# HarborYuan/PolyphonicFormer

Hardware: AMD Instinct MI355X
Metric: frames/sec kernel-update+mask fwd, 1024x2048 N=153 S=3 (higher is better)
Workload: dtype bf16 (feature planes as given; query side: updator half hi/lo bf16, attention / FFN / towers one fp16 plane; one fp16 plane of dynamic kernels, fp16 logits); 1 GPU; cfg2: KernelUpdateIterHead.simple_test_mask_preds, 1024x2048, stride-8 128x256, N=153, S=3, L=133, random-init weights; hip_graph=True, streams=4, feature_input_dtype=bf16, mask_logit_input_dtype=float16, output_dtype=torch.float16, parallelism=frames sharded over 1 GPU(s), no data-path collective

## Files before the change

### polyphonicformer_amd/csrc/ph_convup.hip

```cpp
#include <stdlib.h>

#include <type_traits>

#include "ph_conv_inl.h"

__device__ __forceinline__ void lds_wait_all() {
    asm volatile("s_waitcnt lgkmcnt(0)" ::: "memory");
    __builtin_amdgcn_sched_barrier(0);
}


template <typename OutT> struct UpElem;
template <> struct UpElem<ph_h16> { static constexpr int E = PH_E_F16; };
template <> struct UpElem<uint16_t> { static constexpr int E = PH_E_BF16; };

template <int NRT> struct UpmCfg {
    static constexpr int NW = NRT + 1;
    static constexpr int TILEB = 256 * CONV_T * 2;
    static constexpr int ROWT = 128 + 16;
    static constexpr int TB = 32 * ROWT;
    static constexpr int PATCHB = NRT * 2 * TB;
    static constexpr int KBB = NRT * 32 * 4;
    static constexpr int CONSTB = 6 * 1024;
    static constexpr int NBUF = 3 * TILEB + PATCHB + KBB + CONSTB <= 160 * 1024 ? 3 : 2;
    static constexpr int LDSB = NBUF * TILEB + PATCHB + KBB + CONSTB;
};

template <int OFF> __device__ __forceinline__ void lds_write64_asm(uint32_t byte_addr, uint32_t lo, uint32_t hi) {
    const u32x2_t v = {lo, hi};
    asm volatile("ds_write_b64 %0, %1 offset:%2" ::"v"(byte_addr), "v"(v), "n"(OFF) : "memory");
}

template <int EO> __device__ __forceinline__ uint4 upm_main_frag(int lane, float w) {
    const int opx = lane & 31, g = lane >> 5, j = opx >> 1;
    uint32_t h[8];
#pragma unroll
    for (int e = 0; e < 8; ++e) {
        const int px = (e & 3) + 8 * (e >> 2) + 4 * g;
        float u = 0.f;
        if (px == j) u = 0.75f;
        else if ((opx & 1) ? px == j + 1 : px == j - 1) u = 0.25f;
        h[e] = f2e<EO>(w * u);
    }
    return make_uint4(pack2(h[0], h[1]), pack2(h[2], h[3]), pack2(h[4], h[5]), pack2(h[6], h[7]));
}
template <int EO> __device__ __forceinline__ uint4 upm_edge_frag(int lane, float wP, float wC) {
    const int opx = lane & 31, g = lane >> 5;
    const float l = (g == 0 && opx == 0) ? 0.25f : 0.f, r = (g == 0 && opx == 31) ? 0.25f : 0.f;
    return make_uint4(pack2(f2e<EO>(wP * l), f2e<EO>(wP * r)), pack2(f2e<EO>(wC * l), f2e<EO>(wC * r)), 0u, 0u);
}

template <int E, int NRT, int NTR, bool LOWRES, typename OutT>
__global__ __launch_bounds__(((NRT + 1) * 64)) void k_dynconv_up2m(const uint16_t* __restrict__ planes, const uint16_t* __restrict__ kern,
                                                                  int64_t kern_batch_stride, const float* __restrict__ kbias,
                                                                  int64_t kbias_batch_stride, OutT* __restrict__ logits_out,
                                                                  OutT* __restrict__ up_out, int B, int N, int H) {
    using C = UpmCfg<NRT>;
    constexpr int NBUF = C::NBUF, W = NTR * 64, ROWT = C::ROWT, EO = UpElem<OutT>::E, NH = 2 * NTR;
    constexpr bool COOP = E == PH_E_F16_FROM_BF16;
    extern __shared__ __attribute__((aligned(16))) uint16_t lds[];
    const int tid = threadIdx.x, lane = tid & 63;
    const int wave = __builtin_amdgcn_readfirstlane(tid >> 6);
    const bool producer = wave == NRT;
    const int rt = producer ? 0 : wave;
    const int g = lane >> 5, i16 = lane & 15, gi = (lane >> 4) & 1, ql = lane & 31;
    const int64_t HW = (int64_t)H * W;
    const int ntiles = H * NTR;

    const int64_t rows_total = (int64_t)B * H;
    const int R0 = (int)(rows_total * blockIdx.x / gridDim.x), R1 = (int)(rows_total * (blockIdx.x + 1) / gridDim.x);
    if (R0 >= R1) return;
    const int halo = (R0 % H) != 0 ? 1 : 0;
    const int tg0 = (R0 - halo) * NTR, tg1 = R1 * NTR;

    const uint32_t dma_lane_off = 2u * (uint32_t)((lane >> 3) * HW + (((lane & 7) ^ conv_swz(lane >> 3)) * 8));
    const int64_t row8_bytes = 2 * 8 * HW;
    const int64_t frame_jump = 2 * ((int64_t)PH_C * HW - (int64_t)ntiles * CONV_T);
    int it = tg0 % ntiles, ti = tg0;
    const char* iptr = (const char*)planes + 2 * ((int64_t)(tg0 / ntiles) * PH_C * HW + (int64_t)it * CONV_T);
    auto issue_next = [&](int buf) {
        const char* src = iptr + dma_lane_off;
#pragma unroll
        for (int j = 0; j < 32; ++j)
            __builtin_amdgcn_global_load_lds((const __attribute__((address_space(1))) void*)(src + j * row8_bytes),
                                             (PH_LDS void*)((PH_LDS char*)lds + buf * C::TILEB + j * 1024), 16, 0, PH_CPOL_STREAM);
        ++ti;
        iptr += 2 * CONV_T;
        if (++it == ntiles) { it = 0; iptr += frame_jump; }
    };
    if (producer) {
#pragma unroll
        for (int d = 0; d < NBUF - 1; ++d)
            if (ti < tg1) issue_next(d);
    }

    const int row0 = g * 8 + (i16 >> 2);
    uint32_t frag_off[2];
#pragma unroll
    for (int h = 0; h < 2; ++h) frag_off[h] = 2u * (uint32_t)(row0 * CONV_T + (((h * 4 + gi * 2) ^ conv_swz(row0)) * 8) + (i16 & 3) * 4);
    const uint32_t lds0 = lds_addr(lds);
    const uint32_t tbuf = lds0 + NBUF * C::TILEB + rt * 2 * C::TB;
    float* kb_lds = (float*)((unsigned char*)lds + NBUF * C::TILEB + C::PATCHB) + rt * 32;
    const uint32_t kb_addr = lds_addr(kb_lds) + 4 * ql;
    const uint32_t tw_addr = tbuf + (uint32_t)(ql * ROWT + 8 * g);
    const int sq = lane >> 3, ss = lane & 7;
    const uint32_t tr_addr = tbuf + (uint32_t)(sq * ROWT + 16 * ss);
    const int64_t up_plane = (int64_t)2 * H * 2 * W;
    const uint32_t up_lane_off = 2u * (uint32_t)(sq * up_plane + 8 * ss);
    const int64_t up_kk_bytes = 2 * 8 * up_plane;
    const uint32_t lr_lane_off = 2u * (uint32_t)(sq * HW + 8 * ss);
    const int64_t lr_kk_bytes = 2 * 8 * HW;

    const uint32_t cfrag = lds0 + NBUF * C::TILEB + C::PATCHB + C::KBB + 16u * (uint32_t)lane;
    if (wave == 0) {
        uint4* cw = (uint4*)((unsigned char*)lds + NBUF * C::TILEB + C::PATCHB + C::KBB) + lane;
        cw[0 * 64] = upm_main_frag<EO>(lane, 0.75f);
        cw[1 * 64] = upm_main_frag<EO>(lane, 0.25f);
        cw[2 * 64] = upm_edge_frag<EO>(lane, 0.75f, 0.25f);
        cw[3 * 64] = upm_edge_frag<EO>(lane, 0.25f, 0.75f);
        cw[4 * 64] = upm_main_frag<EO>(lane, 1.0f);
        cw[5 * 64] = upm_edge_frag<EO>(lane, 0.f, 1.0f);
    }
    __syncthreads();

    uint4 af[1][16];
    uint4 prev[NTR][2][2];
#pragma unroll
    for (int a = 0; a < NTR; ++a)
#pragma unroll
        for (int h = 0; h < 2; ++h) { prev[a][h][0] = make_uint4(0, 0, 0, 0); prev[a][h][1] = make_uint4(0, 0, 0, 0); }
    uint4 Cp0 = make_uint4(0, 0, 0, 0), Cp1 = Cp0;
    uint32_t Pe = 0, Ce = 0;

    auto mf = [&](uint4 a, uint4 b, f32x16_t c) -> f32x16_t {
        if constexpr (EO == PH_E_F16) return __builtin_amdgcn_mfma_f32_32x32x16_f16(__builtin_bit_cast(f16x8_t, a), __builtin_bit_cast(f16x8_t, b), c, 0, 0, 0);
        else return mfma32(a, b, c);
    };
    auto xg = [&](uint32_t v) -> uint32_t { return (uint32_t)__shfl_xor((int)v, 32); };
    const f32x16_t zero16 = {0.f, 0.f, 0.f, 0.f, 0.f, 0.f, 0.f, 0.f, 0.f, 0.f, 0.f, 0.f, 0.f, 0.f, 0.f, 0.f};

    auto out_row = [&](auto mp_tag, auto mc_tag, auto me_tag, uint4 P0, uint4 P1, uint4 C0, uint4 C1, uint4 e0, uint4 e1, char* dst_row) {
        constexpr int MP = decltype(mp_tag)::value, MC = decltype(mc_tag)::value, ME = decltype(me_tag)::value;
        uint32_t cf = cfrag;
        asm volatile("" : "+v"(cf));
        u32x4_t kc = lds_read128o_asm<MC * 1024>(cf), ke = lds_read128o_asm<ME * 1024>(cf), kp = kc;
        if constexpr (MP >= 0) kp = lds_read128o_asm<MP * 1024>(cf);
        lds_wait_all();
        const uint4 KC = __builtin_bit_cast(uint4, kc), KE = __builtin_bit_cast(uint4, ke), KP = __builtin_bit_cast(uint4, kp);
        f32x16_t a0 = zero16, a1 = zero16;
        if constexpr (MP >= 0) { a0 = mf(KP, P0, a0); a1 = mf(KP, P1, a1); }
        a0 = mf(KC, C0, a0); a1 = mf(KC, C1, a1);
        a0 = mf(KE, e0, a0); a1 = mf(KE, e1, a1);
        {
            uint32_t w[8];
#pragma unroll
            for (int j = 0; j < 8; ++j) w[j] = f2e_pk<EO>(a0[2 * j], a0[2 * j + 1]);
            lds_write64_asm<0>(tw_addr, w[0], w[1]);  lds_write64_asm<16>(tw_addr, w[2], w[3]);
            lds_write64_asm<32>(tw_addr, w[4], w[5]); lds_write64_asm<48>(tw_addr, w[6], w[7]);
#pragma unroll
            for (int j = 0; j < 8; ++j) w[j] = f2e_pk<EO>(a1[2 * j], a1[2 * j + 1]);
            lds_write64_asm<64>(tw_addr, w[0], w[1]); lds_write64_asm<80>(tw_addr, w[2], w[3]);
            lds_write64_asm<96>(tw_addr, w[4], w[5]); lds_write64_asm<112>(tw_addr, w[6], w[7]);
        }
        lds_wait_all();
        uint32_t tr = tr_addr;
        asm volatile("" : "+v"(tr));
        u32x4_t x[4];
        x[0] = lds_read128o_asm<0 * 8 * ROWT>(tr); x[1] = lds_read128o_asm<1 * 8 * ROWT>(tr);
        x[2] = lds_read128o_asm<2 * 8 * ROWT>(tr); x[3] = lds_read128o_asm<3 * 8 * ROWT>(tr);
        lds_wait_all();
#pragma unroll
        for (int kk = 0; kk < 4; ++kk)
            if (rt * 32 + sq + 8 * kk < N) st_nt16(dst_row + kk * up_kk_bytes + up_lane_off, __builtin_bit_cast(uint4, x[kk]));
    };
    int cur = 0, cur_b = -1;
    for (int gr = R0 - halo; gr < R1; ++gr) {
        const int b = gr / H, r = gr - b * H;
        const bool silent = gr < R0, first = r == 0, last = r == H - 1;
        if (!producer && b != cur_b) {
            const uint16_t* kr = kern + (int64_t)b * kern_batch_stride + (rt * 32 + (lane & 31)) * PH_C + g * 8;
#pragma unroll
            for (int ks = 0; ks < 16; ++ks) af[0][ks] = *(const uint4*)(kr + ks * 16);
            if (lane < 32) kb_lds[lane] = kbias[(int64_t)b * kbias_batch_stride + rt * 32 + lane];
            __builtin_amdgcn_s_waitcnt(0x0F70);
        }
        cur_b = b;
        char* up_row = (char*)(up_out + ((int64_t)b * N + rt * 32) * up_plane + (int64_t)(2 * r) * (2 * W));
        char* lr_row = LOWRES ? (char*)(logits_out + ((int64_t)b * N + rt * 32) * HW + (int64_t)r * W) : nullptr;

        auto emit = [&](auto eh_tag, uint4 P0, uint4 P1, uint4 C0, uint4 C1, uint32_t lP, uint32_t lC, uint32_t rP, uint32_t rC) {
            constexpr int EH = decltype(eh_tag)::value;
            uint32_t l0P, l0C, r1P, r1C;
            if constexpr (EH == 0) { l0P = P0.x & 0xFFFFu; l0C = C0.x & 0xFFFFu; }
            else { l0P = xg(lP) >> 16; l0C = xg(lC) >> 16; }
            if constexpr (EH == NH - 1) { r1P = xg(P1.w) >> 16; r1C = xg(C1.w) >> 16; }
            else { r1P = rP & 0xFFFFu; r1C = rC & 0xFFFFu; }
            const uint32_t p15 = xg(P0.w) >> 16, c15 = xg(C0.w) >> 16;
            const uint32_t keep = g ? 0u : 0xFFFFFFFFu;
            const uint4 e0 = make_uint4((l0P | (P1.x << 16)) & keep, (l0C | (C1.x << 16)) & keep, 0u, 0u);
            const uint4 e1 = make_uint4((p15 | (r1P << 16)) & keep, (c15 | (r1C << 16)) & keep, 0u, 0u);
            char* ub = up_row + 2 * 64 * EH;
            constexpr auto c0 = std::integral_constant<int, 0>{}; constexpr auto c1 = std::integral_constant<int, 1>{};
            constexpr auto c2 = std::integral_constant<int, 2>{}; constexpr auto c3 = std::integral_constant<int, 3>{};
            constexpr auto c4 = std::integral_constant<int, 4>{}; constexpr auto c5 = std::integral_constant<int, 5>{};
            constexpr auto cn = std::integral_constant<int, -1>{};
            if (!first) {
                out_row(c0, c1, c2, P0, P1, C0, C1, e0, e1, ub - 2 * (2 * W));
                out_row(c1, c0, c3, P0, P1, C0, C1, e0, e1, ub);
            } else {
                out_row(cn, c4, c5, P0, P1, C0, C1, e0, e1, ub);
            }
            if (last) out_row(cn, c4, c5, P0, P1, C0, C1, e0, e1, ub + 2 * (2 * W));
        };

        auto tile = [&](auto tc_tag) {
            constexpr int TC = decltype(tc_tag)::value;
            const int tg = gr * NTR + TC;
            if (producer) {
                const int younger = (tg1 - 1 - tg) < (NBUF - 2) ? (tg1 - 1 - tg) : (NBUF - 2);
                if (NBUF >= 3 && younger >= 1) asm volatile("s_waitcnt vmcnt(32)" ::: "memory");
                else asm volatile("s_waitcnt vmcnt(0)" ::: "memory");
            }
            __builtin_amdgcn_s_barrier();
            __builtin_amdgcn_sched_barrier(0);
            if (producer && ti < tg1) {
                int nb = cur + NBUF - 1;
                if (nb >= NBUF) nb -= NBUF;
                issue_next(nb);
            }
            __builtin_amdgcn_sched_barrier(0);
            if constexpr (COOP) {
                constexpr int PIECES = 256 * CONV_T * 2 / 16, LANES = C::NW * 64, ROUNDS = (PIECES + LANES - 1) / LANES;
                const uint32_t tb = lds0 + cur * C::TILEB + 16u * (uint32_t)tid;
                u32x4_t cv[ROUNDS];
#pragma unroll
                for (int q = 0; q < ROUNDS; ++q)
                    if ((q + 1) * LANES <= PIECES || tid < PIECES - q * LANES) cv[q] = lds_read128_asm(tb + q * LANES * 16);
                asm volatile("s_waitcnt lgkmcnt(0)" ::: "memory");
                __builtin_amdgcn_sched_barrier(0);
#pragma unroll
                for (int q = 0; q < ROUNDS; ++q)
                    if ((q + 1) * LANES <= PIECES || tid < PIECES - q * LANES) {
                        const uint4 h16 = bf2h_x8(__builtin_bit_cast(uint4, cv[q]));
                        lds_write128_asm(tb + q * LANES * 16, __builtin_bit_cast(u32x4_t, h16));
                    }
                asm volatile("s_waitcnt lgkmcnt(0)" ::: "memory");
                __builtin_amdgcn_s_barrier();
                __builtin_amdgcn_sched_barrier(0);
            }
            if (!producer) {
                float bl;
                asm volatile("ds_read_b32 %0, %1\n s_waitcnt lgkmcnt(0)" : "=&v"(bl) : "v"(kb_addr) : "memory");
                float bias[16];
#pragma unroll
                for (int q = 0; q < 16; ++q) bias[q] = bl;
#pragma unroll
                for (int h = 0; h < 2; ++h) {
                    const uint32_t fa = lds0 + cur * C::TILEB + frag_off[h];
                    f32x16_t acc;
                    constexpr int KB = 2;
                    u32x2_t bq[2][1][KB][2];
                    conv_read_batch<1, KB, 0>(fa, bq[0]);
                    conv_batches<1, 1, E, KB, 0, true>(fa, af, bq, acc, bias);
                    const uint4 cu0 = make_uint4(f2e_pk<EO>(acc[0], acc[1]), f2e_pk<EO>(acc[2], acc[3]), f2e_pk<EO>(acc[4], acc[5]), f2e_pk<EO>(acc[6], acc[7]));
                    const uint4 cu1 = make_uint4(f2e_pk<EO>(acc[8], acc[9]), f2e_pk<EO>(acc[10], acc[11]), f2e_pk<EO>(acc[12], acc[13]), f2e_pk<EO>(acc[14], acc[15]));
                    if (!silent) {
                        auto body = [&](auto hh_tag) {
                            constexpr int HH = decltype(hh_tag)::value;
                            if constexpr (LOWRES) {
                                asm volatile("s_nop 7" ::: "memory");
                                constexpr int HB = (HH & 1) * 64;
                                lds_write64_asm<C::TB + HB + 0>(tw_addr, cu0.x, cu0.y);  lds_write64_asm<C::TB + HB + 16>(tw_addr, cu0.z, cu0.w);
                                lds_write64_asm<C::TB + HB + 32>(tw_addr, cu1.x, cu1.y); lds_write64_asm<C::TB + HB + 48>(tw_addr, cu1.z, cu1.w);
                                if constexpr ((HH & 1) == 1) {
                                    lds_wait_all();
                                    u32x4_t x[4];
                                    x[0] = lds_read128o_asm<C::TB + 0 * 8 * ROWT>(tr_addr); x[1] = lds_read128o_asm<C::TB + 1 * 8 * ROWT>(tr_addr);
                                    x[2] = lds_read128o_asm<C::TB + 2 * 8 * ROWT>(tr_addr); x[3] = lds_read128o_asm<C::TB + 3 * 8 * ROWT>(tr_addr);
                                    lds_wait_all();
#pragma unroll
                                    for (int kk = 0; kk < 4; ++kk)
                                        if (rt * 32 + sq + 8 * kk < N)
                                            *(uint4*)(lr_row + 2 * 64 * TC + kk * lr_kk_bytes + lr_lane_off) = __builtin_bit_cast(uint4, x[kk]);
                                }
                            }
                            constexpr int TCp = (HH > 0) ? (HH - 1) / 2 : 0, hp = (HH > 0) ? (HH - 1) % 2 : 0;
                            if constexpr (HH > 0) {
                                emit(std::integral_constant<int, HH - 1>{}, prev[TCp][hp][0], prev[TCp][hp][1], Cp0, Cp1, Pe, Ce, prev[TC][h][0].x, cu0.x);
                                Pe = prev[TCp][hp][1].w; Ce = Cp1.w;
                                prev[TCp][hp][0] = Cp0; prev[TCp][hp][1] = Cp1;
                            }
                            if constexpr (HH == NH - 1) {
                                emit(std::integral_constant<int, HH>{}, prev[TC][h][0], prev[TC][h][1], cu0, cu1, Pe, Ce, 0u, 0u);
                                prev[TC][h][0] = cu0; prev[TC][h][1] = cu1;
                            } else {
                                Cp0 = cu0; Cp1 = cu1;
                            }
                        };
                        if (h == 0) body(std::integral_constant<int, 2 * TC>{});
                        else body(std::integral_constant<int, 2 * TC + 1>{});
                    } else {
                        prev[TC][h][0] = cu0; prev[TC][h][1] = cu1;
                    }
                }
            }
            cur = cur + 1 == NBUF ? 0 : cur + 1;
        };
        tile(std::integral_constant<int, 0>{});
        if constexpr (NTR > 1) tile(std::integral_constant<int, 1>{});
        if constexpr (NTR > 2) tile(std::integral_constant<int, 2>{});
        if constexpr (NTR > 3) tile(std::integral_constant<int, 3>{});
    }
}

extern "C" int ph_dynconv_up2_supported(int N, int H, int W, int prec, int out_dtype) {
    if (N <= 64 || N > 224 || H <= 0 || W != 256) return 0;
    if (((int64_t)H * W) % 128) return 0;
    if (prec == PH_PREC_BF16) return out_dtype == PH_OUT_BF16;
    if (prec == PH_PREC_F16 || prec == PH_PREC_BF16_KF16) return out_dtype == PH_OUT_F16;
    return 0;
}

template <int E, int NRT, typename OutT>
static void launch_up(const uint16_t* planes, const uint16_t* kern, int64_t kbs, const float* kbias, int64_t bbs, void* logits_out,
                      void* up_out, int B, int N, int H, int want_wgs, const PhUp2Knobs& kn, hipStream_t s) {
    constexpr int NTR = 4;
    const int64_t rows = (int64_t)B * H;
    int wgs = want_wgs > 0 ? want_wgs : ph_num_cus();
    if (wgs <= 0) wgs = 256;
    if (kn.wgs > 0) wgs = kn.wgs;
    if (wgs > rows) wgs = (int)rows;
    const dim3 grid(wgs), block((NRT + 1) * 64);
    constexpr int lds = UpmCfg<NRT>::LDSB;
#define UP_GO(LR)                                                                                                             \
    do {                                                                                                                      \
        static const bool once = [] {                                                                                         \
            (void)hipFuncSetAttribute((const void*)k_dynconv_up2m<E, NRT, NTR, LR, OutT>, hipFuncAttributeMaxDynamicSharedMemorySize, lds); \
            return true;                                                                                                      \
        }();                                                                                                                  \
        (void)once;                                                                                                           \
        hipLaunchKernelGGL((k_dynconv_up2m<E, NRT, NTR, LR, OutT>), grid, block, lds, s, planes, kern, kbs, kbias, bbs, (OutT*)logits_out, \
                           (OutT*)up_out, B, N, H);                                                                                \
    } while (0)
    if (logits_out) UP_GO(true);
    else UP_GO(false);
#undef UP_GO
}

int ph_dynconv_up2_k(const PhUp2Knobs& kn, const uint16_t* planes, const uint16_t* kern, int64_t kern_batch_stride, const float* kbias,
                     int64_t kbias_batch_stride, void* logits_out, void* up_out, int out_dtype, int B, int N, int H, int W, int prec,
                     int workgroups, void* stream) {
    PH_CHECK_ARG(planes && kern && kbias && up_out && B > 0 && workgroups >= 0, "bad pointer or size");
    if (!ph_dynconv_up2_supported(N, H, W, prec, out_dtype)) {
        ph_set_error("ph_dynconv_up2: unsupported geometry or arithmetic (use ph_dynconv + ph_upsample2x)");
        return PH_EUNSUPPORTED;
    }
    const int nrt = ph_n_padded(N) / 32;
    hipStream_t s = (hipStream_t)stream;
#define UP_ARGS planes, kern, kern_batch_stride, kbias, kbias_batch_stride, logits_out, up_out, B, N, H, workgroups, kn, s
#define UP_CASE(R)                                                                                   \
    case R:                                                                                          \
        if (prec == PH_PREC_BF16) launch_up<PH_E_BF16, R, uint16_t>(UP_ARGS);                        \
        else if (prec == PH_PREC_F16) launch_up<PH_E_F16, R, ph_h16>(UP_ARGS);                       \
        else launch_up<PH_E_F16_FROM_BF16, R, ph_h16>(UP_ARGS);                                      \
        break;
    switch (nrt) {
        UP_CASE(3) UP_CASE(4) UP_CASE(5) UP_CASE(6) UP_CASE(7)
        default: ph_set_error("ph_dynconv_up2: unsupported N"); return PH_EUNSUPPORTED;
    }
#undef UP_CASE
#undef UP_ARGS
    PH_CHECK_LAUNCH();
    return PH_OK;
}

extern "C" int ph_dynconv_up2_wgs(const uint16_t* planes, const uint16_t* kern, int64_t kern_batch_stride, const float* kbias,
                                  int64_t kbias_batch_stride, void* logits_out, void* up_out, int out_dtype, int B, int N, int H, int W,
                                  int prec, int workgroups, void* stream) {
    PhUp2Knobs kn;
    if (const char* e = getenv("PH_UP2_WGS")) kn.wgs = atoi(e) > 0 ? atoi(e) : 0;
    return ph_dynconv_up2_k(kn, planes, kern, kern_batch_stride, kbias, kbias_batch_stride, logits_out, up_out, out_dtype, B, N, H, W, prec,
                            workgroups, stream);
}

extern "C" int ph_dynconv_up2(const uint16_t* planes, const uint16_t* kern, int64_t kern_batch_stride, const float* kbias,
                              int64_t kbias_batch_stride, void* logits_out, void* up_out, int out_dtype, int B, int N, int H, int W,
                              int prec, void* stream) {
    return ph_dynconv_up2_wgs(planes, kern, kern_batch_stride, kbias, kbias_batch_stride, logits_out, up_out, out_dtype, B, N, H, W, prec, 0,
                              stream);
}
```

Before: 16300 frames/s.

## Software-pipeline transpose stores through double-buffered LDS slots in fused dynconv+upsample kernel

Reworks the output path of the fused dynamic-conv + 2x upsample kernel so each row's LDS transpose readback and global store are deferred and overlapped with the next row's MFMA and LDS writes. It uses two alternating LDS slots and partial lgkmcnt waits instead of full drains. It also hoists the constant-fragment LDS reads to once per emit, replaces the xor-32 shuffle with permlane32_swap, and adds a min-2-waves-per-EU launch bound. An NRT=2 instantiation is added for smaller N. The risks are extra register pressure from carried state and subtle ordering hazards in the deferred stores, including a tail flush.

```diff
diff --git a/polyphonicformer_amd/csrc/ph_convup.hip b/polyphonicformer_amd/csrc/ph_convup.hip
--- a/polyphonicformer_amd/csrc/ph_convup.hip
+++ b/polyphonicformer_amd/csrc/ph_convup.hip
@@ -4,8 +4,8 @@
 
 #include "ph_conv_inl.h"
 
-__device__ __forceinline__ void lds_wait_all() {
-    asm volatile("s_waitcnt lgkmcnt(0)" ::: "memory");
+template <int LEFT> __device__ __forceinline__ void lds_wait() {
+    asm volatile("s_waitcnt lgkmcnt(%0)" ::"n"(LEFT) : "memory");
     __builtin_amdgcn_sched_barrier(0);
 }
 
@@ -51,7 +51,7 @@
 }
 
 template <int E, int NRT, int NTR, bool LOWRES, typename OutT>
-__global__ __launch_bounds__(((NRT + 1) * 64)) void k_dynconv_up2m(const uint16_t* __restrict__ planes, const uint16_t* __restrict__ kern,
+__global__ __launch_bounds__(((NRT + 1) * 64), 2) void k_dynconv_up2m(const uint16_t* __restrict__ planes, const uint16_t* __restrict__ kern,
                                                                   int64_t kern_batch_stride, const float* __restrict__ kbias,
                                                                   int64_t kbias_batch_stride, OutT* __restrict__ logits_out,
                                                                   OutT* __restrict__ up_out, int B, int N, int H) {
@@ -95,23 +95,20 @@
     }
 
     const int row0 = g * 8 + (i16 >> 2);
-    uint32_t frag_off[2];
-#pragma unroll
-    for (int h = 0; h < 2; ++h) frag_off[h] = 2u * (uint32_t)(row0 * CONV_T + (((h * 4 + gi * 2) ^ conv_swz(row0)) * 8) + (i16 & 3) * 4);
+    const uint32_t frag_off0 = 2u * (uint32_t)(row0 * CONV_T + (((gi * 2) ^ conv_swz(row0)) * 8) + (i16 & 3) * 4);
     const uint32_t lds0 = lds_addr(lds);
     const uint32_t tbuf = lds0 + NBUF * C::TILEB + rt * 2 * C::TB;
     float* kb_lds = (float*)((unsigned char*)lds + NBUF * C::TILEB + C::PATCHB) + rt * 32;
-    const uint32_t kb_addr = lds_addr(kb_lds) + 4 * ql;
+    const uint32_t kb_base = lds_addr(kb_lds);
     const uint32_t tw_addr = tbuf + (uint32_t)(ql * ROWT + 8 * g);
     const int sq = lane >> 3, ss = lane & 7;
     const uint32_t tr_addr = tbuf + (uint32_t)(sq * ROWT + 16 * ss);
     const int64_t up_plane = (int64_t)2 * H * 2 * W;
-    const uint32_t up_lane_off = 2u * (uint32_t)(sq * up_plane + 8 * ss);
+    const uint32_t sq_hw2 = 2u * (uint32_t)(sq * HW);
     const int64_t up_kk_bytes = 2 * 8 * up_plane;
-    const uint32_t lr_lane_off = 2u * (uint32_t)(sq * HW + 8 * ss);
     const int64_t lr_kk_bytes = 2 * 8 * HW;
 
-    const uint32_t cfrag = lds0 + NBUF * C::TILEB + C::PATCHB + C::KBB + 16u * (uint32_t)lane;
+    const uint32_t cfrag_base = lds0 + NBUF * C::TILEB + C::PATCHB + C::KBB;
     if (wave == 0) {
         uint4* cw = (uint4*)((unsigned char*)lds + NBUF * C::TILEB + C::PATCHB + C::KBB) + lane;
         cw[0 * 64] = upm_main_frag<EO>(lane, 0.75f);
@@ -136,81 +133,137 @@
         if constexpr (EO == PH_E_F16) return __builtin_amdgcn_mfma_f32_32x32x16_f16(__builtin_bit_cast(f16x8_t, a), __builtin_bit_cast(f16x8_t, b), c, 0, 0, 0);
         else return mfma32(a, b, c);
     };
-    auto xg = [&](uint32_t v) -> uint32_t { return (uint32_t)__shfl_xor((int)v, 32); };
+    auto xg = [&](uint32_t v) -> uint32_t {
+        const auto sw = __builtin_amdgcn_permlane32_swap(v, v, false, false);
+        return g ? sw[0] : sw[1];
+    };
     const f32x16_t zero16 = {0.f, 0.f, 0.f, 0.f, 0.f, 0.f, 0.f, 0.f, 0.f, 0.f, 0.f, 0.f, 0.f, 0.f, 0.f, 0.f};
 
-    auto out_row = [&](auto mp_tag, auto mc_tag, auto me_tag, uint4 P0, uint4 P1, uint4 C0, uint4 C1, uint4 e0, uint4 e1, char* dst_row) {
-        constexpr int MP = decltype(mp_tag)::value, MC = decltype(mc_tag)::value, ME = decltype(me_tag)::value;
-        uint32_t cf = cfrag;
-        asm volatile("" : "+v"(cf));
-        u32x4_t kc = lds_read128o_asm<MC * 1024>(cf), ke = lds_read128o_asm<ME * 1024>(cf), kp = kc;
-        if constexpr (MP >= 0) kp = lds_read128o_asm<MP * 1024>(cf);
-        lds_wait_all();
-        const uint4 KC = __builtin_bit_cast(uint4, kc), KE = __builtin_bit_cast(uint4, ke), KP = __builtin_bit_cast(uint4, kp);
+    constexpr int ROW_UP = 0, ROW_LR = 1;
+    int pend_lim = 0;
+    char* pend_dst = (char*)up_out;
+    uint32_t wslot = 0;
+    auto pend_load = [&](u32x4_t (&x)[4]) {
+        uint32_t tr = tr_addr + (C::TB - wslot);
+        asm volatile("" : "+v"(tr));
+        x[0] = lds_read128o_asm<0 * 8 * ROWT>(tr); x[1] = lds_read128o_asm<1 * 8 * ROWT>(tr);
+        x[2] = lds_read128o_asm<2 * 8 * ROWT>(tr); x[3] = lds_read128o_asm<3 * 8 * ROWT>(tr);
+    };
+    auto pend_store = [&](auto kind_tag, const u32x4_t (&x)[4]) {
+        constexpr int KIND = decltype(kind_tag)::value;
+        int ln = lane;
+        asm volatile("" : "+v"(ln));
+        const int psq = ln >> 3;
+        const uint32_t off = (KIND == ROW_UP ? 4u * sq_hw2 : sq_hw2) + 16u * (uint32_t)(ln & 7);
+#pragma unroll
+        for (int kk = 0; kk < 4; ++kk)
+            if (rt * 32 + psq + 8 * kk < pend_lim) {
+                if constexpr (KIND == ROW_UP) st_nt16(pend_dst + kk * up_kk_bytes + off, __builtin_bit_cast(uint4, x[kk]));
+                else *(uint4*)(pend_dst + kk * lr_kk_bytes + off) = __builtin_bit_cast(uint4, x[kk]);
+            }
+    };
+    auto pend_set = [&](char* dst) { pend_dst = dst; pend_lim = N; wslot = C::TB - wslot; };
+
+    auto up_job = [&](auto conly_tag, auto pend_kind, uint4 KP, uint4 KC, uint4 KE, uint4 P0, uint4 P1, uint4 C0, uint4 C1, uint4 e0, uint4 e1,
+                      char* dst_row) {
+        constexpr bool CONLY = decltype(conly_tag)::value;
         f32x16_t a0 = zero16, a1 = zero16;
-        if constexpr (MP >= 0) { a0 = mf(KP, P0, a0); a1 = mf(KP, P1, a1); }
+        if constexpr (!CONLY) { a0 = mf(KP, P0, a0); a1 = mf(KP, P1, a1); }
         a0 = mf(KC, C0, a0); a1 = mf(KC, C1, a1);
         a0 = mf(KE, e0, a0); a1 = mf(KE, e1, a1);
-        {
-            uint32_t w[8];
-#pragma unroll
-            for (int j = 0; j < 8; ++j) w[j] = f2e_pk<EO>(a0[2 * j], a0[2 * j + 1]);
-            lds_write64_asm<0>(tw_addr, w[0], w[1]);  lds_write64_asm<16>(tw_addr, w[2], w[3]);
-            lds_write64_asm<32>(tw_addr, w[4], w[5]); lds_write64_asm<48>(tw_addr, w[6], w[7]);
-#pragma unroll
-            for (int j = 0; j < 8; ++j) w[j] = f2e_pk<EO>(a1[2 * j], a1[2 * j + 1]);
-            lds_write64_asm<64>(tw_addr, w[0], w[1]); lds_write64_asm<80>(tw_addr, w[2], w[3]);
-            lds_write64_asm<96>(tw_addr, w[4], w[5]); lds_write64_asm<112>(tw_addr, w[6], w[7]);
-        }
-        lds_wait_all();
-        uint32_t tr = tr_addr;
-        asm volatile("" : "+v"(tr));
+        __builtin_amdgcn_sched_barrier(0);
+        uint32_t tw = tw_addr + wslot;
+        asm volatile("" : "+v"(tw));
+        uint32_t w[8];
+#pragma unroll
+        for (int j = 0; j < 8; ++j) w[j] = f2e_pk<EO>(a0[2 * j], a0[2 * j + 1]);
+        lds_write64_asm<0>(tw, w[0], w[1]);  lds_write64_asm<16>(tw, w[2], w[3]);
+        lds_write64_asm<32>(tw, w[4], w[5]); lds_write64_asm<48>(tw, w[6], w[7]);
+        lds_wait<4>();
         u32x4_t x[4];
-        x[0] = lds_read128o_asm<0 * 8 * ROWT>(tr); x[1] = lds_read128o_asm<1 * 8 * ROWT>(tr);
-        x[2] = lds_read128o_asm<2 * 8 * ROWT>(tr); x[3] = lds_read128o_asm<3 * 8 * ROWT>(tr);
-        lds_wait_all();
-#pragma unroll
-        for (int kk = 0; kk < 4; ++kk)
-            if (rt * 32 + sq + 8 * kk < N) st_nt16(dst_row + kk * up_kk_bytes + up_lane_off, __builtin_bit_cast(uint4, x[kk]));
+        pend_load(x);
+#pragma unroll
+        for (int j = 0; j < 8; ++j) w[j] = f2e_pk<EO>(a1[2 * j], a1[2 * j + 1]);
+        lds_write64_asm<64>(tw, w[0], w[1]); lds_write64_asm<80>(tw, w[2], w[3]);
+        lds_write64_asm<96>(tw, w[4], w[5]); lds_write64_asm<112>(tw, w[6], w[7]);
+        __builtin_amdgcn_sched_barrier(0);
+        lds_wait<4>();
+        pend_store(pend_kind, x);
+        pend_set(dst_row);
+    };
+    auto lr_job = [&](uint4 A0, uint4 A1, uint4 B0, uint4 B1, char* dst_row) {
+        u32x4_t x[4];
+        lds_wait<0>();
+        pend_load(x);
+        uint32_t tw = tw_addr + wslot;
+        asm volatile("" : "+v"(tw));
+        lds_write64_asm<0>(tw, A0.x, A0.y);  lds_write64_asm<16>(tw, A0.z, A0.w);
+        lds_write64_asm<32>(tw, A1.x, A1.y); lds_write64_asm<48>(tw, A1.z, A1.w);
+        lds_write64_asm<64>(tw, B0.x, B0.y); lds_write64_asm<80>(tw, B0.z, B0.w);
+        lds_write64_asm<96>(tw, B1.x, B1.y); lds_write64_asm<112>(tw, B1.z, B1.w);
+        lds_wait<8>();
+        pend_store(std::integral_constant<int, ROW_UP>{}, x);
+        pend_set(dst_row);
     };
     int cur = 0, cur_b = -1;
     for (int gr = R0 - halo; gr < R1; ++gr) {
         const int b = gr / H, r = gr - b * H;
         const bool silent = gr < R0, first = r == 0, last = r == H - 1;
         if (!producer && b != cur_b) {
-            const uint16_t* kr = kern + (int64_t)b * kern_batch_stride + (rt * 32 + (lane & 31)) * PH_C + g * 8;
+            int ln = lane;
+            asm volatile("" : "+v"(ln));
+            const uint16_t* kr = kern + (int64_t)b * kern_batch_stride + (rt * 32 + (ln & 31)) * PH_C + (ln >> 5) * 8;
 #pragma unroll
             for (int ks = 0; ks < 16; ++ks) af[0][ks] = *(const uint4*)(kr + ks * 16);
-            if (lane < 32) kb_lds[lane] = kbias[(int64_t)b * kbias_batch_stride + rt * 32 + lane];
+            if (ln < 32) kb_lds[ln] = kbias[(int64_t)b * kbias_batch_stride + rt * 32 + ln];
             __builtin_amdgcn_s_waitcnt(0x0F70);
         }
         cur_b = b;
         char* up_row = (char*)(up_out + ((int64_t)b * N + rt * 32) * up_plane + (int64_t)(2 * r) * (2 * W));
         char* lr_row = LOWRES ? (char*)(logits_out + ((int64_t)b * N + rt * 32) * HW + (int64_t)r * W) : nullptr;
 
-        auto emit = [&](auto eh_tag, uint4 P0, uint4 P1, uint4 C0, uint4 C1, uint32_t lP, uint32_t lC, uint32_t rP, uint32_t rC) {
+        auto emit = [&](auto eh_tag, auto pk_tag, uint4 P0, uint4 P1, uint4 C0, uint4 C1, uint32_t lP, uint32_t lC, uint32_t rP, uint32_t rC) {
             constexpr int EH = decltype(eh_tag)::value;
-            uint32_t l0P, l0C, r1P, r1C;
-            if constexpr (EH == 0) { l0P = P0.x & 0xFFFFu; l0C = C0.x & 0xFFFFu; }
-            else { l0P = xg(lP) >> 16; l0C = xg(lC) >> 16; }
-            if constexpr (EH == NH - 1) { r1P = xg(P1.w) >> 16; r1C = xg(C1.w) >> 16; }
-            else { r1P = rP & 0xFFFFu; r1C = rC & 0xFFFFu; }
-            const uint32_t p15 = xg(P0.w) >> 16, c15 = xg(C0.w) >> 16;
-            const uint32_t keep = g ? 0u : 0xFFFFFFFFu;
-            const uint4 e0 = make_uint4((l0P | (P1.x << 16)) & keep, (l0C | (C1.x << 16)) & keep, 0u, 0u);
-            const uint4 e1 = make_uint4((p15 | (r1P << 16)) & keep, (c15 | (r1C << 16)) & keep, 0u, 0u);
+            auto edges = [&](uint4& e0, uint4& e1) {
+                uint32_t l0P, l0C, r1P, r1C;
+                if constexpr (EH == 0) { l0P = P0.x & 0xFFFFu; l0C = C0.x & 0xFFFFu; }
+                else { l0P = xg(lP) >> 16; l0C = xg(lC) >> 16; }
+                if constexpr (EH == NH - 1) { r1P = xg(P1.w) >> 16; r1C = xg(C1.w) >> 16; }
+                else { r1P = rP & 0xFFFFu; r1C = rC & 0xFFFFu; }
+                const uint32_t p15 = xg(P0.w) >> 16, c15 = xg(C0.w) >> 16;
+                const uint32_t keep = g ? 0u : 0xFFFFFFFFu;
+                e0 = make_uint4((l0P | (P1.x << 16)) & keep, (l0C | (C1.x << 16)) & keep, 0u, 0u);
+                e1 = make_uint4((p15 | (r1P << 16)) & keep, (c15 | (r1C << 16)) & keep, 0u, 0u);
+            };
             char* ub = up_row + 2 * 64 * EH;
-            constexpr auto c0 = std::integral_constant<int, 0>{}; constexpr auto c1 = std::integral_constant<int, 1>{};
-            constexpr auto c2 = std::integral_constant<int, 2>{}; constexpr auto c3 = std::integral_constant<int, 3>{};
-            constexpr auto c4 = std::integral_constant<int, 4>{}; constexpr auto c5 = std::integral_constant<int, 5>{};
-            constexpr auto cn = std::integral_constant<int, -1>{};
+            constexpr auto both = std::false_type{}; constexpr auto conly = std::true_type{};
+            constexpr auto pk_up = std::integral_constant<int, ROW_UP>{};
+            auto edge_of = [](u32x4_t k) { return make_uint4(k.x, k.y, 0u, 0u); };
+            int ln = lane;
+            asm volatile("" : "+v"(ln));
+            const uint32_t cfrag = cfrag_base + 16u * (uint32_t)ln;
+            uint4 e0, e1;
             if (!first) {
-                out_row(c0, c1, c2, P0, P1, C0, C1, e0, e1, ub - 2 * (2 * W));
-                out_row(c1, c0, c3, P0, P1, C0, C1, e0, e1, ub);
-            } else {
-                out_row(cn, c4, c5, P0, P1, C0, C1, e0, e1, ub);
-            }
-            if (last) out_row(cn, c4, c5, P0, P1, C0, C1, e0, e1, ub + 2 * (2 * W));
+                const u32x4_t k0 = lds_read128o_asm<0 * 1024>(cfrag), k1 = lds_read128o_asm<1 * 1024>(cfrag);
+                const u32x4_t k2 = lds_read128o_asm<2 * 1024>(cfrag), k3 = lds_read128o_asm<3 * 1024>(cfrag);
+                edges(e0, e1);
+                lds_wait<0>();
+                const uint4 K0 = __builtin_bit_cast(uint4, k0), K1 = __builtin_bit_cast(uint4, k1);
+                up_job(both, pk_tag, K0, K1, edge_of(k2), P0, P1, C0, C1, e0, e1, ub - 2 * (2 * W));
+                up_job(both, pk_up, K1, K0, edge_of(k3), P0, P1, C0, C1, e0, e1, ub);
+            }
+            if (first || last) {
+                const u32x4_t k4 = lds_read128o_asm<4 * 1024>(cfrag), k5 = lds_read128o_asm<5 * 1024>(cfrag);
+                if (first) edges(e0, e1);
+                lds_wait<0>();
+                const uint4 K4 = __builtin_bit_cast(uint4, k4);
+                if (first) {
+                    up_job(conly, pk_tag, K4, K4, edge_of(k5), P0, P1, C0, C1, e0, e1, ub);
+                    if (last) up_job(conly, pk_up, K4, K4, edge_of(k5), P0, P1, C0, C1, e0, e1, ub + 2 * (2 * W));
+                } else {
+                    up_job(conly, pk_up, K4, K4, edge_of(k5), P0, P1, C0, C1, e0, e1, ub + 2 * (2 * W));
+                }
+            }
         };
 
         auto tile = [&](auto tc_tag) {
@@ -250,13 +303,16 @@
             }
             if (!producer) {
                 float bl;
+                int ln = lane;
+                asm volatile("" : "+v"(ln));
+                const uint32_t kb_addr = kb_base + 4u * (uint32_t)(ln & 31);
                 asm volatile("ds_read_b32 %0, %1\n s_waitcnt lgkmcnt(0)" : "=&v"(bl) : "v"(kb_addr) : "memory");
                 float bias[16];
 #pragma unroll
                 for (int q = 0; q < 16; ++q) bias[q] = bl;
 #pragma unroll
                 for (int h = 0; h < 2; ++h) {
-                    const uint32_t fa = lds0 + cur * C::TILEB + frag_off[h];
+                    const uint32_t fa = lds0 + cur * C::TILEB + (frag_off0 ^ (h ? 64u : 0u));
                     f32x16_t acc;
                     constexpr int KB = 2;
                     u32x2_t bq[2][1][KB][2];
@@ -267,31 +323,18 @@
                     if (!silent) {
                         auto body = [&](auto hh_tag) {
                             constexpr int HH = decltype(hh_tag)::value;
-                            if constexpr (LOWRES) {
-                                asm volatile("s_nop 7" ::: "memory");
-                                constexpr int HB = (HH & 1) * 64;
-                                lds_write64_asm<C::TB + HB + 0>(tw_addr, cu0.x, cu0.y);  lds_write64_asm<C::TB + HB + 16>(tw_addr, cu0.z, cu0.w);
-                                lds_write64_asm<C::TB + HB + 32>(tw_addr, cu1.x, cu1.y); lds_write64_asm<C::TB + HB + 48>(tw_addr, cu1.z, cu1.w);
-                                if constexpr ((HH & 1) == 1) {
-                                    lds_wait_all();
-                                    u32x4_t x[4];
-                                    x[0] = lds_read128o_asm<C::TB + 0 * 8 * ROWT>(tr_addr); x[1] = lds_read128o_asm<C::TB + 1 * 8 * ROWT>(tr_addr);
-                                    x[2] = lds_read128o_asm<C::TB + 2 * 8 * ROWT>(tr_addr); x[3] = lds_read128o_asm<C::TB + 3 * 8 * ROWT>(tr_addr);
-                                    lds_wait_all();
-#pragma unroll
-                                    for (int kk = 0; kk < 4; ++kk)
-                                        if (rt * 32 + sq + 8 * kk < N)
-                                            *(uint4*)(lr_row + 2 * 64 * TC + kk * lr_kk_bytes + lr_lane_off) = __builtin_bit_cast(uint4, x[kk]);
-                                }
-                            }
+                            constexpr bool LR_NOW = LOWRES && (HH & 1) == 1;
+                            if constexpr (LR_NOW) lr_job(Cp0, Cp1, cu0, cu1, lr_row + 2 * 64 * TC);
                             constexpr int TCp = (HH > 0) ? (HH - 1) / 2 : 0, hp = (HH > 0) ? (HH - 1) % 2 : 0;
                             if constexpr (HH > 0) {
-                                emit(std::integral_constant<int, HH - 1>{}, prev[TCp][hp][0], prev[TCp][hp][1], Cp0, Cp1, Pe, Ce, prev[TC][h][0].x, cu0.x);
+                                emit(std::integral_constant<int, HH - 1>{}, std::integral_constant<int, LR_NOW ? ROW_LR : ROW_UP>{}, prev[TCp][hp][0],
+                                     prev[TCp][hp][1], Cp0, Cp1, Pe, Ce, prev[TC][h][0].x, cu0.x);
                                 Pe = prev[TCp][hp][1].w; Ce = Cp1.w;
                                 prev[TCp][hp][0] = Cp0; prev[TCp][hp][1] = Cp1;
                             }
                             if constexpr (HH == NH - 1) {
-                                emit(std::integral_constant<int, HH>{}, prev[TC][h][0], prev[TC][h][1], cu0, cu1, Pe, Ce, 0u, 0u);
+                                emit(std::integral_constant<int, HH>{}, std::integral_constant<int, ROW_UP>{}, prev[TC][h][0], prev[TC][h][1], cu0, cu1,
+                                     Pe, Ce, 0u, 0u);
                                 prev[TC][h][0] = cu0; prev[TC][h][1] = cu1;
                             } else {
                                 Cp0 = cu0; Cp1 = cu1;
@@ -311,14 +354,25 @@
         if constexpr (NTR > 2) tile(std::integral_constant<int, 2>{});
         if constexpr (NTR > 3) tile(std::integral_constant<int, 3>{});
     }
-}
-
-extern "C" int ph_dynconv_up2_supported(int N, int H, int W, int prec, int out_dtype) {
-    if (N <= 64 || N > 224 || H <= 0 || W != 256) return 0;
+    if (!producer) {
+        u32x4_t x[4];
+        lds_wait<0>();
+        pend_load(x);
+        lds_wait<0>();
+        pend_store(std::integral_constant<int, ROW_UP>{}, x);
+    }
+}
+
+static int up2_instantiated(int N, int H, int W, int prec, int out_dtype) {
+    if (N <= 32 || N > 224 || H <= 0 || W != 256) return 0;
     if (((int64_t)H * W) % 128) return 0;
     if (prec == PH_PREC_BF16) return out_dtype == PH_OUT_BF16;
     if (prec == PH_PREC_F16 || prec == PH_PREC_BF16_KF16) return out_dtype == PH_OUT_F16;
     return 0;
+}
+
+extern "C" int ph_dynconv_up2_supported(int N, int H, int W, int prec, int out_dtype) {
+    return N > 64 && up2_instantiated(N, H, W, prec, out_dtype);
 }
 
 template <int E, int NRT, typename OutT>
@@ -351,7 +405,7 @@
                      int64_t kbias_batch_stride, void* logits_out, void* up_out, int out_dtype, int B, int N, int H, int W, int prec,
                      int workgroups, void* stream) {
     PH_CHECK_ARG(planes && kern && kbias && up_out && B > 0 && workgroups >= 0, "bad pointer or size");
-    if (!ph_dynconv_up2_supported(N, H, W, prec, out_dtype)) {
+    if (!up2_instantiated(N, H, W, prec, out_dtype)) {
         ph_set_error("ph_dynconv_up2: unsupported geometry or arithmetic (use ph_dynconv + ph_upsample2x)");
         return PH_EUNSUPPORTED;
     }
@@ -365,7 +419,7 @@
         else launch_up<PH_E_F16_FROM_BF16, R, ph_h16>(UP_ARGS);                                      \
         break;
     switch (nrt) {
-        UP_CASE(3) UP_CASE(4) UP_CASE(5) UP_CASE(6) UP_CASE(7)
+        UP_CASE(2) UP_CASE(3) UP_CASE(4) UP_CASE(5) UP_CASE(6) UP_CASE(7)
         default: ph_set_error("ph_dynconv_up2: unsupported N"); return PH_EUNSUPPORTED;
     }
 #undef UP_CASE
```

After: 16360 frames/s, median of 6. No clear change (+0.4%).
